# Kyaw-Thiha/animal-vision

Hardware: AMD Instinct MI355X
Metric: megapixels/sec per-frame pipeline (higher is better)
Workload: dtype f16

## Files before the change

animal-vision_amd/_lib.py:

```python
from __future__ import annotations

import ctypes
import os

_HERE = os.path.dirname(os.path.abspath(__file__))
LIB_PATH = os.path.join(_HERE, "libavx.so")

AVX_OK = 0
AVX_ERR_INVALID, AVX_ERR_NO_DEVICE, AVX_ERR_HIP, AVX_ERR_UNSUPPORTED, AVX_ERR_NOMEM = -1, -2, -3, -4, -5
AVX_COLOR_MATRIX, AVX_COLOR_CAT_MERGE = 0, 1
AVX_POST_NONE, AVX_POST_GAUSS, AVX_POST_ROWGAIN, AVX_POST_STREAK = 0, 1, 2, 3
AVX_MAX_KSIZE = 33
AVX_PIX_FMTS = {"yuv420p": 0, "nv12": 1, "yuv422p": 2, "yuv444p": 3, "gray": 4, "yuv420p10le": 5, "yuv422p10le": 6, "yuv444p10le": 7,
                "p010le": 8}
AVX_TRANSFERS = {"pq": 1, "hlg": 2}
AVX_TONEMAPS = {"clip": 0, "mobius": 1}


class AvxError(RuntimeError):
    def __init__(self, code: int, msg: str):
        super().__init__(f"libavx error {code}: {msg}")
        self.code = code


# ... 387 lines not shown
                           _vp, _vp, _vp]),
    "avx_remap_linear_planes": (_i, [_vp, _vp, _i, _i, _i, _vp, _vp, _vp, ctypes.c_float, _vp]),
    "avx_sobel3_plane": (_i, [_vp, _vp, _i, _i, _vp, _vp, _vp]),
    "avx_mst_gram": (_i, [_vp, _vp, _i, _sz, _i, _i, _vp, _vp, _vp, _vp]),
    "avx_mst_qkv_gram": (_i, [_vp, _vp, _vp, _sz, _i, _vp, _vp, _vp, _vp, _vp]),
    "avx_mst_qkv_gram16": (_i, [_vp, _vp, _vp, _sz, _i, _vp, _vp, _vp, _vp, _vp]),
    "avx_mst_ln_gemm_gelu": (_i, [_vp, _vp, _vp, _vp, ctypes.c_float, _vp, _sz, _i, _vp, _vp]),
    "avx_mst_convt2x2": (_i, [_vp, _vp, _vp, _vp, _vp, _i, _i, _i, _i, _vp]),
    "avx_mst_convt2x2_fuse": (_i, [_vp, _vp, _vp, _vp, _vp, _vp, _vp, _i, _i, _i, _i, _vp]),
    "avx_mst_posemb": (_i, [_vp, _vp, _vp, _vp, _vp, _vp, _vp, _i, _i, _i, _i, _vp]),
    "avx_mst_conv3x3_add": (_i, [_vp, _vp, _vp, _vp, _vp, _i, _i, _i, _i, _vp]),
    "avx_mst_attn_pack": (_i, [_vp, _vp, _vp, _vp, _vp, _vp, _i, _vp, _vp]),
    "avx_mst_rowgemm_add": (_i, [_vp, _vp, _vp, _vp, _vp, _vp, _vp, _sz, _i, _vp]),
    "avx_mst_conv_in_u8": (_i, [_vp, _vp, _i, _i, _i, _i, _i, _i, _vp, _vp, _vp]),
    "avx_mst_conv3x3_lds": (_i, [_vp, _vp, _vp, _vp, _vp, _i, _i, _i, _i, _vp]),
    "avx_mst_down4x4": (_i, [_vp, _vp, _vp, _vp, _i, _i, _i, _i, _vp]),
    "avx_mst_conv3x3_lds_gram": (_i, [_vp, _vp, _vp, _vp, _vp, _i, _i, _i, _vp, _vp, _vp, _vp, _vp]),
    "avx_mst_conv3x3_lds_cin": (_i, [_vp, _vp, _vp, _vp, _i, _i, _i, _i, _i, _i, _vp, _vp, _vp]),
    "avx_mst_conv3x3_lds_spectral_cin": (_i, [_vp, _vp, _vp, _vp, _i, _i, _i, _i, _i, _i, _vp, _fp, _i, _i, _i, _i, _vp, _vp, ctypes.POINTER(ctypes.c_int), _vp]),
    "avx_mst_conv3x3_lds_gram_cin": (_i, [_vp, _vp, _i, _i, _i, _i, _i, _i, _vp, _vp, _vp, _vp, _vp, _vp, _vp, _vp]),
    "avx_mst_convt2x2_fuse_gram": (_i, [_vp, _vp, _vp, _vp, _vp, _vp, _vp, _i, _i, _i, _vp, _vp, _vp, _vp, _vp]),
    "avx_mst_convt2x2_fuse16": (_i, [_vp, _vp, _vp, _vp, _vp, _vp, _vp, _i, _i, _i, _i, _vp]),
    "avx_mst_convt2x2_fuse16_gram": (_i, [_vp, _vp, _vp, _vp, _vp, _vp, _vp, _i, _i, _i, _i, _vp, _vp, _vp, _vp, _vp]),
    "avx_mst_attn_pack16": (_i, [_vp, _vp, _vp, _vp, _vp, _vp, _i, _vp, _vp]),
    "avx_mst_attn_pack_mx": (_i, [_vp, _vp, _vp, _vp, _vp, _vp, _i, _vp, _vp]),
    "avx_mst_attn_tail_mx": (_i, [_vp, _vp, _vp, _vp, _vp, _vp, _vp, _vp, _i, _i, _i, _i, _vp]),
    "avx_mst_attn_tail_sp": (_i, [_vp, _vp, _vp, _vp, _vp, _vp, _vp, _vp, _i, _i, _i, _i, _vp]),
    "avx_mst_attn_tail_mx_col": (_i, [_vp, _vp, _vp, _vp, _vp, _vp, _vp, _vp, _i, _i, _i, _i, _i, _vp]),
    "avx_mst_attn_tail_sp_col": (_i, [_vp, _vp, _vp, _vp, _vp, _vp, _vp, _vp, _i, _i, _i, _i, _i, _vp]),
    "avx_mst_tail_march_steps": (_i, [_i, _i, _i, _i, ctypes.POINTER(ctypes.c_longlong), ctypes.POINTER(ctypes.c_ubyte), _i, ctypes.POINTER(ctypes.c_int)]),
    "avx_mst_attn_tail": (_i, [_vp, _vp, _vp, _vp, _vp, _vp, _vp, _vp, _i, _i, _i, _i, _vp]),
    "avx_mst_attn_tail_x": (_i, [_vp, _vp, _vp, _vp, _vp, _vp, _vp, _vp, _i, _i, _i, _i, _vp]),
    "avx_mst_ffn_fused": (_i, [_vp, _vp, _vp, _vp, ctypes.c_float, _vp, _vp, _vp, _vp, _i, _i, _i, _i, _vp]),
    "avx_mst_conv3x3_lds_spectral": (_i, [_vp, _vp, _vp, _vp, _i, _i, _i, _fp, _i, _i, _i, _i, _vp, _vp, ctypes.POINTER(ctypes.c_int), _vp]),
    "avx_mst_ffn_fused_mx": (_i, [_vp, _vp, _vp, _vp, ctypes.c_float, _vp, _vp, _vp, _vp, _i, _i, _i, _i, _vp]),
    "avx_mst_ffn_fused_sp": (_i, [_vp, _vp, _vp, _vp, ctypes.c_float, _vp, _vp, _vp, _vp, _i, _i, _i, _i, _vp]),
    "avx_mst_ffn_fused_mx_col": (_i, [_vp, _vp, _vp, _vp, ctypes.c_float, _vp, _vp, _vp, _vp, _i, _i, _i, _i, _i, _vp]),
    "avx_mst_ffn_fused_sp_col": (_i, [_vp, _vp, _vp, _vp, ctypes.c_float, _vp, _vp, _vp, _vp, _i, _i, _i, _i, _i, _vp]),
    "avx_mst_gelu_prescale": (ctypes.c_float, []),
    "avx_mst_tile_order": (_i, [_i, _i, _i, _i, _i, ctypes.POINTER(ctypes.c_longlong), _i, ctypes.POINTER(ctypes.c_int)]),
    "avx_mst_tile_order_col": (_i, [_i, _i, _i, _i, ctypes.POINTER(ctypes.c_longlong), ctypes.POINTER(ctypes.c_ubyte), _i, ctypes.POINTER(ctypes.c_int)]),
    "avx_mst_dw_gemm_add": (_i, [_vp, _vp, _vp, _vp, _vp, _vp, _i, _i, _i, _i, _vp]),
    "avx_dwconv3x3_nhwc_add": (_i, [_vp, _vp, _vp, _vp, _i, _i, _i, _i, _i, _vp, _vp, _vp]),
    "avx_dwconv3x3_nhwc": (_i, [_vp, _vp, _vp, _vp, _i, _i, _i, _i, _i, _i, _vp]),
    "avx_layernorm_rows": (_i, [_vp, _vp, _vp, _vp, _vp, _i, _sz, _i, ctypes.c_float, _vp]),
    "avx_layernorm_rows_grouped": (_i, [_vp, _vp, _vp, _vp, _vp, _i, _sz, _i, ctypes.c_float, _i, _i, _vp]),
# ... 9 lines not shown
```

animal-vision_amd/csrc/mst_mfma.hip:

```cpp
#include <hip/hip_fp16.h>

#include "avx_internal.h"
#include "mst_common.h"

namespace {

constexpr int kT = 256;

__device__ __forceinline__ float16_t mfma(half4_t a, half4_t b, float16_t c) { return __builtin_amdgcn_mfma_f32_32x32x8f16(a, b, c, 0, 0, 0); }
__device__ __forceinline__ float16_t mfma16(half8_t a, half8_t b, float16_t c) { return __builtin_amdgcn_mfma_f32_32x32x16_f16(a, b, c, 0, 0, 0); }

template <int C>
__device__ __forceinline__ void load_x(const __half* __restrict__ x, size_t tile, size_t n, int lane, half4_t (&xf)[C / 8]) {
    const int p = lane & 31, h = lane >> 5;
    const size_t row = tile * 32 + p;
    if (row < n) {
        const uint4* src = reinterpret_cast<const uint4*>(x + row * (size_t)C + h * (C / 2));
#pragma unroll
        for (int q = 0; q < C / 16; ++q) {
            const uint4 v = src[q];
            const half8_t h8 = __builtin_bit_cast(half8_t, v);
            xf[2 * q] = half4_t{h8[0], h8[1], h8[2], h8[3]};
            xf[2 * q + 1] = half4_t{h8[4], h8[5], h8[6], h8[7]};
        }
    } else {
#pragma unroll
// ... 880 lines not shown

template <int C, bool SKIP, bool GRAM>
int launch_convt16(avx_ctx* ctx, avx_ws* ws, const void* x, const void* wpack, const float* bias, const void* skip, const void* wskip, void* out, int B, int H, int W,
                   const void* wqk, float* gram, float* nq, float* nk, hipStream_t s) {
    constexpr int NW = convt16_geom<C, SKIP, GRAM>::NW, KS = C / 16, CO = C / 2, NT = CO / 32, KSS = CO / 16, HD = NT;
    size_t lds = sizeof(uint4) * ((size_t)4 * NT * KS * 64 + (SKIP ? NT * KSS * 64 : 0) + (GRAM ? 2 * HD * KSS * 64 : 0)) + sizeof(float) * CO;
    if (GRAM && lds < sizeof(float) * NW * HD * 34 * 32) lds = sizeof(float) * NW * HD * 34 * 32;
    const long total = (long)B * H * ((W + 31) / 32);
    long blocks = (total + NW - 1) / NW;
    const long cap = (long)ctx->num_cus * convt16_geom<C, SKIP, GRAM>::PER_CU;
    if (blocks > cap) blocks = cap;
    float* partial = nullptr;
    if (GRAM) {
        int rc = avx_ensure_scratch(ctx, ws, sizeof(float) * (size_t)blocks * HD * 34 * 32);
        if (rc) return rc;
        partial = (float*)ws->d_scratch;
    }
    auto k = k_mst_convt2x2_16<C, NW, SKIP, GRAM>;
    AVX_HIP(ctx, hipFuncSetAttribute((const void*)k, hipFuncAttributeMaxDynamicSharedMemorySize, (int)lds));
    hipLaunchKernelGGL(k, dim3((unsigned)blocks), dim3(64 * NW), lds, s, (const __half*)x, (const uint4*)wpack, bias, (const __half*)skip, (const uint4*)wskip, (__half*)out, B,
                       H, W, (const uint4*)wqk, partial);
    AVX_HIP(ctx, hipGetLastError());
    if (GRAM) return avx_mst_qkv_final_launch(ctx, partial, (int)blocks, HD, gram, nq, nk, s);
    return AVX_OK;
}

template <int C, int NW>
__global__ __launch_bounds__(64 * NW) void k_mst_qkv16(const __half* __restrict__ x, const uint4* __restrict__ wpack , size_t n,
                                                      __half* __restrict__ v_out , float* __restrict__ partial ) {
    constexpr int KS = C / 16, HD = C / 32, NT = 3 * HD;
    extern __shared__ __align__(16) unsigned char smem[];
    uint4* wl = reinterpret_cast<uint4*>(smem);
    const int tid = threadIdx.x, lane = tid & 63, wave = tid >> 6;
    for (int i = tid; i < NT * KS * 64; i += 64 * NW) wl[i] = wpack[i];
    __syncthreads();
    auto W = [&](int t, int s) { return __builtin_bit_cast(half8_t, wl[(t * KS + s) * 64 + lane]); };
    float16_t G[HD];
    float nq[HD], nk[HD];
#pragma unroll
    for (int hd = 0; hd < HD; ++hd) {
#pragma unroll
        for (int v = 0; v < 16; ++v) G[hd][v] = 0.f;
        nq[hd] = 0.f;
        nk[hd] = 0.f;
    }
    const size_t ntiles = (n + 31) / 32;
// ... 371 lines not shown
    if (C == 64) {
        if (skip) return launch_convt16<64, true, false>(ctx, nullptr, x, wpack16, bias, skip, wskip16, out, B, H, W, nullptr, nullptr, nullptr, nullptr, s);
        return launch_convt16<64, false, false>(ctx, nullptr, x, wpack16, bias, nullptr, nullptr, out, B, H, W, nullptr, nullptr, nullptr, nullptr, s);
    }
    if (skip) return launch_convt16<128, true, false>(ctx, nullptr, x, wpack16, bias, skip, wskip16, out, B, H, W, nullptr, nullptr, nullptr, nullptr, s);
    return launch_convt16<128, false, false>(ctx, nullptr, x, wpack16, bias, nullptr, nullptr, out, B, H, W, nullptr, nullptr, nullptr, nullptr, s);
}

int avx_mst_convt2x2_fuse16_gram(avx_ctx* ctx, const void* x, const void* wpack16, const float* bias, const void* skip, const void* wskip16, void* out, int H, int W,
                                 int C, int heads, const void* wqk16, float* gram, float* nq, float* nk, void* stream) {
    if (!ctx) return AVX_ERR_INVALID;
    AVX_REQUIRE(ctx, x && wpack16 && bias && skip && wskip16 && out && wqk16 && gram && nq && nk && H > 0 && W > 0, "avx_mst_convt2x2_fuse16_gram: NULL pointer or empty tensor");
    AVX_REQUIRE(ctx, (C == 64 || C == 128) && heads == C / 64, "avx_mst_convt2x2_fuse16_gram: C=%d, heads=%d (64 or 128 input channels, one head per 32 output channels)", C, heads);
    AVX_REQUIRE(ctx, ((((uintptr_t)x | (uintptr_t)wpack16 | (uintptr_t)out | (uintptr_t)skip | (uintptr_t)wskip16 | (uintptr_t)wqk16)) & 15u) == 0,
                "avx_mst_convt2x2_fuse16_gram: pointers must be 16-byte aligned");
    AVX_HIP(ctx, hipSetDevice(ctx->device));
    hipStream_t s = avx_pick_stream(ctx, stream);
    avx_ws* ws = avx_workspace(ctx, s);
    if (!ws) return AVX_ERR_NOMEM;
    if (C == 64) return launch_convt16<64, true, true>(ctx, ws, x, wpack16, bias, skip, wskip16, out, 1, H, W, wqk16, gram, nq, nk, s);
    return launch_convt16<128, true, true>(ctx, ws, x, wpack16, bias, skip, wskip16, out, 1, H, W, wqk16, gram, nq, nk, s);
}

}
```

animal-vision_amd/ml/mst_plus_plus.py:

```python
from __future__ import annotations

from typing import Dict, List

import torch
import torch.nn.functional as F

DIM = 31
PAD = 32


def padded(n: int) -> int:
    assert n % DIM == 0
    return n // DIM * PAD


def pad_index(n: int, device=None) -> torch.Tensor:
    i = torch.arange(n, device=device)
    return (i // DIM) * PAD + i % DIM


def pad_channels(t: torch.Tensor, dims) -> torch.Tensor:
    for d in dims:
        n = t.shape[d]
        shape = list(t.shape)
# ... 138 lines not shown
        self._conv_in = os.environ.get("AVX_MST_NO_CONV_IN", "") == ""
        self._upfuse = os.environ.get("AVX_MST_NO_UPFUSE", "") == ""
        self._tail = os.environ.get("AVX_MST_NO_TAIL", "") == ""
        self._tailx = os.environ.get("AVX_MST_NO_TAILX", "") == ""
        self._down = os.environ.get("AVX_MST_NO_DOWN4X4", "") == ""
        self._qkv16 = os.environ.get("AVX_MST_NO_QKV16", "") == ""
        self._convgram = os.environ.get("AVX_MST_NO_CONVGRAM", "") == ""
        self._ffn = os.environ.get("AVX_MST_NO_FFN_FUSED", "") == ""
        self._gelu_pre = None
        self._dwmx = os.environ.get("AVX_MST_NO_DW_MFMA", "") == ""
        self._dwsp = os.environ.get("AVX_MST_NO_DW_SPARSE", "") == ""
        self.DW_SPARSE_FFN_C = (32, 64, 128)
        self.DW_SPARSE_TAIL_C = (32, 64)
        self._specfuse = os.environ.get("AVX_MST_NO_SPEC_FUSE", "") == ""
        self._cinfuse = os.environ.get("AVX_MST_NO_CONV_IN_FUSE", "") == ""
        self.FFN_FUSED_C = tuple(int(v) for v in os.environ.get("AVX_MST_FFN_FUSED_C", "32,64,128").split(",") if v)
        self._ffn_march = os.environ.get("AVX_MST_NO_FFN_MARCH", "") == ""
        self.FFN_MARCH_C = (32, 64)
        self._tail_march = os.environ.get("AVX_MST_NO_TAIL_MARCH", "") == ""
        self.TAIL_MARCH_C = (32, 64)
        self._convt16 = os.environ.get("AVX_MST_NO_CONVT16", "") == ""
        self.CONVT16_C = (64, 128)
        self.CONVT16_GRAM_C = (128,)
        self._ctx = {}

    def ctx(self, device: torch.device):
        from ..runtime import get_context

        idx = device.index if device.index is not None else torch.cuda.current_device()
        c = get_context(idx)
        if c.device != idx:
            raise RuntimeError(f"libavx context is on device {c.device}, tensor on cuda:{idx} (one process per GPU)")
        return c

    @staticmethod
    def _dt(t: torch.Tensor) -> int:
        if t.dtype == torch.float32:
            return 0
        if t.dtype == torch.float16:
            return 1
        raise TypeError(f"csrc/mst.hip kernels take float32/float16, got {t.dtype}")

    def gram(self, qkv: torch.Tensor, heads: int):
        from .._lib import lib

        b, n, c3 = qkv.shape
# ... 56 lines not shown
            ctx._check(lib.avx_mst_convt2x2(ctx._h, x.data_ptr(), wpack.data_ptr(), bias.data_ptr(), out.data_ptr(), b, h, w, c, st))
        else:
            assert skip.is_contiguous() and skip.shape == out.shape
            ctx._check(lib.avx_mst_convt2x2_fuse(ctx._h, x.data_ptr(), wpack.data_ptr(), bias.data_ptr(), skip.data_ptr(), wskip.data_ptr(), out.data_ptr(), b, h, w, c, st))
        return out

    def convt2x2_gram(self, x: torch.Tensor, wpack: torch.Tensor, bias: torch.Tensor, skip: torch.Tensor, wskip: torch.Tensor, wqk16: torch.Tensor):
        from .._lib import lib

        b, h, w, c = x.shape
        assert c == 64 and skip.is_contiguous() and skip.shape == (b, 2 * h, 2 * w, 32)
        x = x.contiguous()
        out = torch.empty((b, 2 * h, 2 * w, 32), dtype=torch.float16, device=x.device)
        g = torch.empty((b, 1, 32, 32), dtype=torch.float32, device=x.device)
        nq = torch.empty((b, 32), dtype=torch.float32, device=x.device)
        nk = torch.empty((b, 32), dtype=torch.float32, device=x.device)
        ctx = self.ctx(x.device)
        st = torch.cuda.current_stream(x.device).cuda_stream
        for i in range(b):
            ctx._check(lib.avx_mst_convt2x2_fuse_gram(ctx._h, x[i].data_ptr(), wpack.data_ptr(), bias.data_ptr(), skip[i].data_ptr(), wskip.data_ptr(), out[i].data_ptr(), h, w, c,
                                                      wqk16.data_ptr(), g[i].data_ptr(), nq[i].data_ptr(), nk[i].data_ptr(), st))
        return out, g, nq, nk

    def convt2x2_16(self, x: torch.Tensor, wpack16: torch.Tensor, bias: torch.Tensor, skip: torch.Tensor = None, wskip16: torch.Tensor = None) -> torch.Tensor:
        from .._lib import lib

        b, h, w, c = x.shape
        x = x.contiguous()
        out = torch.empty((b, 2 * h, 2 * w, c // 2), dtype=torch.float16, device=x.device)
        ctx = self.ctx(x.device)
        st = torch.cuda.current_stream(x.device).cuda_stream
        if skip is not None:
            assert skip.is_contiguous() and skip.shape == out.shape and wskip16 is not None
        ctx._check(lib.avx_mst_convt2x2_fuse16(ctx._h, x.data_ptr(), wpack16.data_ptr(), bias.data_ptr(), skip.data_ptr() if skip is not None else None,
                                               wskip16.data_ptr() if skip is not None else None, out.data_ptr(), b, h, w, c, st))
        return out

    def convt2x2_16_gram(self, x: torch.Tensor, wpack16: torch.Tensor, bias: torch.Tensor, skip: torch.Tensor, wskip16: torch.Tensor, wqk16: torch.Tensor):
        from .._lib import lib

        b, h, w, c = x.shape
        ch, heads = c // 2, c // 64
        assert c in (64, 128) and skip.is_contiguous() and skip.shape == (b, 2 * h, 2 * w, ch)
        x = x.contiguous()
        out = torch.empty((b, 2 * h, 2 * w, ch), dtype=torch.float16, device=x.device)
        g = torch.empty((b, heads, 32, 32), dtype=torch.float32, device=x.device)
        nq = torch.empty((b, ch), dtype=torch.float32, device=x.device)
        nk = torch.empty((b, ch), dtype=torch.float32, device=x.device)
        ctx = self.ctx(x.device)
        st = torch.cuda.current_stream(x.device).cuda_stream
        for i in range(b):
            ctx._check(lib.avx_mst_convt2x2_fuse16_gram(ctx._h, x[i].data_ptr(), wpack16.data_ptr(), bias.data_ptr(), skip[i].data_ptr(), wskip16.data_ptr(), out[i].data_ptr(),
                                                        h, w, c, heads, wqk16.data_ptr(), g[i].data_ptr(), nq[i].data_ptr(), nk[i].data_ptr(), st))
        return out, g, nq, nk

    def posemb(self, v: torch.Tensor, w1_c9: torch.Tensor, w2_c9: torch.Tensor, residual: torch.Tensor = None, bias: torch.Tensor = None) -> torch.Tensor:
        from .._lib import lib

        b, h, w, c = v.shape
        v = v.contiguous()
        residual = residual.contiguous() if residual is not None else None
        out = torch.empty_like(v)
        ctx = self.ctx(v.device)
        ctx._check(lib.avx_mst_posemb(ctx._h, v.data_ptr(), w1_c9.data_ptr(), w2_c9.data_ptr(), residual.data_ptr() if residual is not None else None,
                                      bias.data_ptr() if bias is not None else None, out.data_ptr(), b, h, w, c, torch.cuda.current_stream(v.device).cuda_stream))
        return out

    def conv3x3(self, x: torch.Tensor, wpack: torch.Tensor, add: torch.Tensor = None) -> torch.Tensor:
        from .._lib import lib

        b, h, w, c = x.shape
        x = x.contiguous()
        add = add.contiguous() if add is not None else None
        out = torch.empty_like(x)
        ctx = self.ctx(x.device)
        ctx._check(lib.avx_mst_conv3x3_add(ctx._h, x.data_ptr(), wpack.data_ptr(), add.data_ptr() if add is not None else None, out.data_ptr(), b, h, w, c,
# ... 551 lines not shown
            fea = self._conv3(x, ekey)
        skips: List[torch.Tensor] = []
        heads = 1
        for i in range(2):
            fea = self._msab(fea, f"{p}.encoder_layers.{i}.0", heads, pre if i == 0 else None)
            skips.append(fea)
            dkey = f"{p}.encoder_layers.{i}.1.weight"
            if _AVX.fused_ok(fea) and _AVX._down and fea.shape[-1] in (32, 64) and fea.is_contiguous():
                fea = _AVX.down4x4(fea, self._prep(dkey + ".frag16", lambda: pack_down4x4(self._w(dkey, (0, 1)))))
            else:
                fea = self._conv_nhwc(fea, self._w(dkey, (0, 1)), stride=2, padding=1)
            heads *= 2
        fea = self._msab(fea, p + ".bottleneck", heads)
        for i in range(2):
            kw = f"{p}.decoder_layers.{i}.0.weight"
            if _AVX.fused_ok(fea) and fea.shape[-1] in (64, 128) and _AVX._upfuse:
                ch = fea.shape[-1] // 2
                wfk = f"{p}.fuse{i}"
                wf_ = self._prep(wfk, lambda: self._w(f"{p}.decoder_layers.{i}.1.weight", (0, 1)).reshape(ch, 2 * ch).t().contiguous())
                gb = self._prep(kw + ".upfuse.bias", lambda: (self._w(f"{p}.decoder_layers.{i}.0.bias", (0,)).float() @ wf_[:ch].float()).contiguous())
                heads //= 2
                a2 = f"{p}.decoder_layers.{i}.2.blocks.0.0"
                cangram = _AVX._convgram and _AVX._qkv16 and _AVX._tail and _AVX._tailx
                gram16 = cangram and _AVX._convt16 and 2 * ch in _AVX.CONVT16_C and 2 * ch in _AVX.CONVT16_GRAM_C
                gram8 = cangram and ch == 32 and not gram16
                k16 = gram16 or (_AVX._convt16 and 2 * ch in _AVX.CONVT16_C and not gram8)
                tap = lambda t: (self._w(kw, (0, 1))[:, :, t // 2, t % 2].float() @ wf_[:ch].float()).half().contiguous()
                if k16:
                    gt = self._prep(kw + ".upfuse4k16", lambda: torch.stack([pack_fragments16(tap(t), halfrow=True) for t in range(4)]).contiguous())
                    wbot_ = self._prep(f"{p}.fuse{i}.bot16", lambda: pack_fragments16(wf_[ch:].contiguous(), halfrow=True))
                else:
                    gt = self._prep(kw + ".upfuse4", lambda: torch.stack([pack_fragments(tap(t), True) for t in range(4)]).contiguous())
                    wbot_ = self._prep(f"{p}.fuse{i}.bot", lambda: pack_fragments(wf_[ch:].contiguous(), True))
                pre2 = None
                if gram16 or gram8:
                    wqkv2 = self._prep(a2 + ".qkv", lambda: torch.cat([self._w(a2 + ".to_q.weight", (0, 1)), self._w(a2 + ".to_k.weight", (0, 1)),
                                                                       self._w(a2 + ".to_v.weight", (0, 1))], 0).t().contiguous())
                    wqk2 = self._prep(a2 + ".qkv.frag16", lambda: pack_qkv16(wqkv2))
                    fea, *pre2 = (_AVX.convt2x2_16_gram if gram16 else _AVX.convt2x2_gram)(fea, gt, gb, skips[1 - i].contiguous(), wbot_, wqk2)
                else:
                    fea = (_AVX.convt2x2_16 if k16 else _AVX.convt2x2)(fea, gt, gb, skips[1 - i].contiguous(), wbot_)
                fea = self._msab(fea, f"{p}.decoder_layers.{i}.2", heads, tuple(pre2) if pre2 else None)
                continue
            if _AVX.fused_ok(fea) and fea.shape[-1] in (64, 128):
                wt = self._prep(kw + ".frag4", lambda: torch.stack([pack_fragments(self._w(kw, (0, 1))[:, :, t // 2, t % 2].contiguous(), True) for t in range(4)]).contiguous())
                bt = self._prep(kw + ".bias32", lambda: self._w(f"{p}.decoder_layers.{i}.0.bias", (0,)).float().contiguous())
                up = _AVX.convt2x2(fea, wt, bt)
            else:
                up = F.conv_transpose2d(fea.permute(0, 3, 1, 2), self._w(kw, (0, 1)), self._w(f"{p}.decoder_layers.{i}.0.bias", (0,)), stride=2).permute(0, 2, 3, 1)
            heads //= 2
            skip = skips[1 - i]
            b, h, w, ch = up.shape
            c2 = 2 * ch
            wf = self._prep(f"{p}.fuse{i}", lambda: self._w(f"{p}.decoder_layers.{i}.1.weight", (0, 1)).reshape(c2 // 2, c2).t().contiguous())
            if _AVX.fused_ok(skip):
                up, skip = up.contiguous(), skip.contiguous()
                wtop = self._prep(f"{p}.fuse{i}.top", lambda: pack_fragments(wf[:ch].contiguous(), True))
                wbot = self._prep(f"{p}.fuse{i}.bot", lambda: pack_fragments(wf[ch:].contiguous(), True))
                fea = _AVX.rowgemm_add(up.reshape(b * h * w, ch), wtop, None, skip.reshape(b * h * w, ch), wbot).reshape(b, h, w, ch)
            else:
                cat = torch.cat([up, skip], dim=-1)
                fea = (cat.reshape(b, h * w, c2) @ wf).reshape(b, h, w, c2 // 2)
            fea = self._msab(fea, f"{p}.decoder_layers.{i}.2", heads)
        if src is not None:
# ... 91 lines not shown
```

include/avx.h:

```cpp
#ifndef AVX_H
#define AVX_H

#include <stddef.h>
#include <stdint.h>

#ifdef __cplusplus
extern "C" {
#endif

#define AVX_ABI_VERSION 1

typedef struct avx_ctx avx_ctx;

typedef enum avx_status {
    AVX_OK = 0,
    AVX_ERR_INVALID = -1,
    AVX_ERR_NO_DEVICE = -2,
    AVX_ERR_HIP = -3,
    AVX_ERR_UNSUPPORTED = -4,
    AVX_ERR_NOMEM = -5
} avx_status;

int avx_abi_version(void);
int avx_device_count(void);
// ... 459 lines not shown
                             const float* bias, void* out, int B, int H, int W, int C, int max_workgroups, void* stream);
int avx_mst_attn_tail_sp_col(avx_ctx* ctx, const void* x, const void* wvpack16, const void* mpack_mx, const void* dw1pack, const void* dw2pack,
                             const float* bias, void* out, int B, int H, int W, int C, int max_workgroups, void* stream);
int avx_mst_tail_march_steps(int frames, int ty, int tx, int nwg, long long* visit, unsigned char* prime, int steps_cap, int* steps_out);

int avx_mst_rowgemm_add(avx_ctx* ctx, const void* a, const void* wpack, const void* a2, const void* wpack2, const void* add, void* out, size_t rows,
                        int C, void* stream);

int avx_mst_attn_pack(avx_ctx* ctx, const float* gram, const float* nq, const float* nk, const float* rescale, const float* wproj_t, int C,
                      void* mpack, void* stream);

int avx_mst_conv3x3_add(avx_ctx* ctx, const void* x, const void* wpack, const void* add, void* out, int B, int H, int W, int C, void* stream);

int avx_mst_posemb(avx_ctx* ctx, const void* v, const float* w1_c9, const float* w2_c9, const void* residual, const float* bias, void* out, int B,
                   int H, int W, int C, void* stream);

int avx_mst_convt2x2(avx_ctx* ctx, const void* x, const void* wpack, const float* bias, void* out, int B, int H, int W, int C, void* stream);
int avx_mst_convt2x2_fuse(avx_ctx* ctx, const void* x, const void* wpack, const float* bias, const void* skip, const void* wskip, void* out, int B, int H,
                          int W, int C, void* stream);
int avx_mst_convt2x2_fuse16(avx_ctx* ctx, const void* x, const void* wpack16, const float* bias, const void* skip, const void* wskip16, void* out, int B, int H,
                            int W, int C, void* stream);
int avx_mst_convt2x2_fuse16_gram(avx_ctx* ctx, const void* x, const void* wpack16, const float* bias, const void* skip, const void* wskip16, void* out, int H, int W,
                                 int C, int heads, const void* wqk16, float* gram, float* nq, float* nk, void* stream);

int avx_dwconv3x3_nhwc(avx_ctx* ctx, const void* x, const float* w_c9, void* y, int dtype, int B, int H, int W, int C, int gelu_out, void* stream);
int avx_dwconv3x3_nhwc_add(avx_ctx* ctx, const void* x, const float* w_c9, void* y, int B, int H, int W, int C, int gelu_out,
                           const void* residual, const float* bias, void* stream);

int avx_layernorm_rows(avx_ctx* ctx, const void* x, const float* gamma, const float* beta, void* y, int dtype, size_t rows, int C, float eps, void* stream);
int avx_layernorm_rows_grouped(avx_ctx* ctx, const void* x, const float* gamma, const float* beta, void* y, int dtype, size_t rows, int C, float eps,
                               int group, int real, void* stream);

int avx_get_table(int which, void* dst_host, size_t capacity);

#ifdef __cplusplus
}
#endif
#endif
```

Measured before the change: 464.6.

## Add whole-line convt2x2 fuse kernel with async skip DMA into LDS

Adds a new transposed-conv 2x2 fused kernel that processes whole output line runs per wave. It streams the skip input with global_load_lds DMA into swizzled LDS areas, double-buffered across tiles. Results are staged in LDS so the global stores are fully coalesced, and a variant also fuses the gram/qkv reduction for C=64. This targets uncoalesced skip reads and output writes and overlaps memory with MFMA work. In exchange it uses one large workgroup per CU, inline asm waitcnt tricks and complex swizzle maps.

```diff
diff --git a/animal-vision_amd/_lib.py b/animal-vision_amd/_lib.py
--- a/animal-vision_amd/_lib.py
+++ b/animal-vision_amd/_lib.py
@@ -433,6 +433,9 @@
     "avx_mst_convt2x2_fuse_gram": (_i, [_vp, _vp, _vp, _vp, _vp, _vp, _vp, _i, _i, _i, _vp, _vp, _vp, _vp, _vp]),
     "avx_mst_convt2x2_fuse16": (_i, [_vp, _vp, _vp, _vp, _vp, _vp, _vp, _i, _i, _i, _i, _vp]),
     "avx_mst_convt2x2_fuse16_gram": (_i, [_vp, _vp, _vp, _vp, _vp, _vp, _vp, _i, _i, _i, _i, _vp, _vp, _vp, _vp, _vp]),
+    "avx_mst_convt2x2_fuse16_ln": (_i, [_vp, _vp, _vp, _vp, _vp, _vp, _vp, _i, _i, _i, _i, _vp]),
+    "avx_mst_convt2x2_fuse16_gram_ln": (_i, [_vp, _vp, _vp, _vp, _vp, _vp, _vp, _i, _i, _i, _i, _vp, _vp, _vp, _vp, _vp]),
+    "avx_mst_convt_lines_map": (_i, [_i] + [ctypes.POINTER(ctypes.c_int)] * 4),
     "avx_mst_attn_pack16": (_i, [_vp, _vp, _vp, _vp, _vp, _vp, _i, _vp, _vp]),
     "avx_mst_attn_pack_mx": (_i, [_vp, _vp, _vp, _vp, _vp, _vp, _i, _vp, _vp]),
     "avx_mst_attn_tail_mx": (_i, [_vp, _vp, _vp, _vp, _vp, _vp, _vp, _vp, _i, _i, _i, _i, _vp]),
diff --git a/animal-vision_amd/csrc/mst_convt_lines.h b/animal-vision_amd/csrc/mst_convt_lines.h
--- /dev/null
+++ b/animal-vision_amd/csrc/mst_convt_lines.h
@@ -0,0 +1,26 @@
+#pragma once
+
+__host__ __device__ constexpr int convt_ln_skip_slot(int cpp, int i, int k) {
+    if (cpp == 4) {
+        const int ql = k >> 2, c = k & 3, hi = ql >> 3, pl = (ql >> 1) & 3, dx = ql & 1;
+        return 16 * c + 4 * ((i ^ (3 * hi) ^ dx) & 3) + pl;
+    }
+    const int ql = k >> 3, c = k & 7, pl = ql >> 1, dx = ql & 1;
+    return 16 * (c >> 1) + 4 * ((i & 3) ^ (2 * (c & 1) + dx)) + pl;
+}
+__host__ __device__ constexpr int convt_ln_skip_chunk(int cpp, int i, int l) {
+    const int u = l >> 4, v = ((l >> 2) ^ i) & 3, pl = l & 3;
+    if (cpp == 4) {
+        const int hi = v >> 1, dx = (v & 1) ^ hi;
+        return 4 * (8 * hi + 2 * pl + dx) + u;
+    }
+    return 8 * (2 * pl + (v & 1)) + 2 * u + (v >> 1);
+}
+__host__ __device__ constexpr int convt_ln_operand_byte(int cpp, int p, int h, int dx, int s) {
+    const int g = (2 * p + dx) * cpp + h * (cpp / 2) + s;
+    return 1024 * (g >> 6) + 16 * convt_ln_skip_slot(cpp, g >> 6, g & 63);
+}
+__host__ __device__ constexpr int convt_ln_out_byte(int cpp, int g) {
+    const int i = g >> 6, k = g & 63;
+    return 1024 * i + 16 * (k ^ (cpp == 4 ? k >> 3 : ((k >> 4) & 3) | (i & 1) << 2));
+}
diff --git a/animal-vision_amd/csrc/mst_mfma.hip b/animal-vision_amd/csrc/mst_mfma.hip
--- a/animal-vision_amd/csrc/mst_mfma.hip
+++ b/animal-vision_amd/csrc/mst_mfma.hip
@@ -2,6 +2,7 @@
 
 #include "avx_internal.h"
 #include "mst_common.h"
+#include "mst_convt_lines.h"
 
 namespace {
 
@@ -928,6 +929,253 @@
                        H, W, (const uint4*)wqk, partial);
     AVX_HIP(ctx, hipGetLastError());
     if (GRAM) return avx_mst_qkv_final_launch(ctx, partial, (int)blocks, HD, gram, nq, nk, s);
+    return AVX_OK;
+}
+
+#pragma clang diagnostic push
+#pragma clang diagnostic ignored "-Winline-asm"
+__device__ __forceinline__ void ln_dma16(const void* base , unsigned ofs, unsigned lds_base ) {
+    asm volatile("s_mov_b32 m0, %0\n\ts_nop 0\n\tglobal_load_lds_dwordx4 %1, %2" ::"s"(__builtin_amdgcn_readfirstlane(lds_base)), "v"(ofs), "s"(base) : "memory", "m0");
+}
+#pragma clang diagnostic pop
+template <int C, bool GRAM> struct convt_ln_geom {
+    static constexpr int NW = C == 128 ? 8 : GRAM ? 12 : 16, AREAS = C == 128 ? 1 : 2, KS = C / 16, CO = C / 2, NT = CO / 32, KSS = CO / 16, HD = NT, NP = C / 16, ROWB = 64 * C;
+    static constexpr int WBYTES = 16 * (4 * NT * KS * 64 + NT * KSS * 64 + (GRAM ? 2 * HD * KSS * 64 : 0)) + 4 * CO;
+    static constexpr int LDS = (WBYTES + 1023) / 1024 * 1024 + 1024  + NW * AREAS * ROWB;
+    static_assert(LDS <= 160 * 1024 && (!GRAM || 4 * NW * HD * 34 * 32 <= LDS), "one workgroup per CU");
+};
+template <int C, int NW_, bool GRAM>
+__global__ __launch_bounds__(64 * NW_, 1) void k_mst_convt2x2_16_ln(const __half* __restrict__ x , const uint4* __restrict__ wpack ,
+                                                                  const float* __restrict__ bias , const __half* __restrict__ skip ,
+                                                                  const uint4* __restrict__ wskip , __half* __restrict__ out , int B,
+                                                                  int H, int W, const uint4* __restrict__ wqk , float* __restrict__ partial ) {
+    using G_ = convt_ln_geom<C, GRAM>;
+    static_assert(NW_ == G_::NW, "the geometry is convt_ln_geom's");
+    constexpr int NW = G_::NW, AREAS = G_::AREAS, KS = G_::KS, CO = G_::CO, NT = G_::NT, KSS = G_::KSS, HD = G_::HD, NP = G_::NP, ROWB = G_::ROWB;
+    using run_t = unsigned __attribute__((ext_vector_type(4 * NP)));
+    using u4_t = unsigned __attribute__((ext_vector_type(4)));
+    extern __shared__ __align__(16) unsigned char smem[];
+    uint4* wl = reinterpret_cast<uint4*>(smem);
+    float* bl = reinterpret_cast<float*>(wl + 4 * NT * KS * 64);
+    uint4* wsl = reinterpret_cast<uint4*>(bl + CO);
+    uint4* wq = wsl + NT * KSS * 64;
+    const int tid = threadIdx.x, lane = tid & 63, wave = __builtin_amdgcn_readfirstlane(tid >> 6);
+    for (int i = tid; i < 4 * NT * KS * 64; i += 64 * NW) wl[i] = wpack[i];
+    for (int i = tid; i < CO; i += 64 * NW) bl[i] = bias[i];
+    for (int i = tid; i < NT * KSS * 64; i += 64 * NW) wsl[i] = wskip[i];
+    float16_t G[GRAM ? HD : 1];
+    float nq[GRAM ? HD : 1], nk[GRAM ? HD : 1];
+    if constexpr (GRAM) {
+        for (int i = tid; i < 2 * HD * KSS * 64; i += 64 * NW) wq[i] = wqk[i];
+#pragma unroll
+        for (int hd = 0; hd < HD; ++hd) {
+#pragma unroll
+            for (int v = 0; v < 16; ++v) G[hd][v] = 0.f;
+            nq[hd] = 0.f;
+            nk[hd] = 0.f;
+        }
+    }
+    __syncthreads();
+    const int xt = (W + 31) / 32;
+    const unsigned total = (unsigned)B * (unsigned)H * (unsigned)xt;
+    const int p = lane & 31, h = lane >> 5;
+    const unsigned lds0 = (unsigned)(size_t)(__attribute__((address_space(3))) unsigned char*)smem;
+    const unsigned a0 = __builtin_amdgcn_readfirstlane(((lds0 + (unsigned)G_::WBYTES + 1023u) & ~1023u) + (unsigned)wave * (AREAS * ROWB));
+    unsigned char* const area = smem + (a0 - lds0);
+    int fo[NP], ob[2][KSS], wb[2][NT][2];
+    const int rb[2] = {convt_ln_out_byte(NP, lane), convt_ln_out_byte(NP, 64 + lane) - 1024};
+#pragma unroll
+    for (int i = 0; i < NP; ++i) fo[i] = 1024 * i + 16 * convt_ln_skip_chunk(NP, i, lane);
+#pragma unroll
+    for (int dx = 0; dx < 2; ++dx) {
+#pragma unroll
+        for (int s = 0; s < KSS; ++s) ob[dx][s] = convt_ln_operand_byte(NP, p, h, dx, s);
+#pragma unroll
+        for (int t = 0; t < NT; ++t) {
+            wb[dx][t][0] = convt_ln_out_byte(NP, (2 * p + dx) * NP + 4 * t + 2 * h);
+            wb[dx][t][1] = convt_ln_out_byte(NP, (2 * p + dx) * NP + 4 * t + 2 * h + 1);
+        }
+    }
+    const unsigned nwaves = gridDim.x * NW, first = blockIdx.x * NW + wave;
+    const int sx = (int)(nwaves % (unsigned)xt), sy = (int)(nwaves / (unsigned)xt);
+    int xi = (int)(first % (unsigned)xt), yb = (int)(first / (unsigned)xt);
+    unsigned tile = first;
+    auto run_ofs = [&](int yb_, int xi_, int dy) { return ((size_t)(2 * yb_ + dy) * (size_t)(2 * W) + (size_t)(64 * xi_)) * (size_t)C; };
+    auto run_len = [&](int xi_) { const int px = 2 * W - 64 * xi_; return (px < 64 ? px : 64) * C; };
+    auto request = [&](int yb_, int xi_, int dy, int a) {
+        const char* base = reinterpret_cast<const char*>(skip) + run_ofs(yb_, xi_, dy);
+        const int last = run_len(xi_) - 16;
+#pragma unroll
+        for (int i = 0; i < NP; ++i) ln_dma16(base, (unsigned)(fo[i] < last ? fo[i] : last), a0 + a * ROWB + i * 1024);
+    };
+    auto load_x = [&](int yb_, int xi_, u4_t (&r)[KS]) {
+        const int xw = 32 * xi_ + p;
+        const u4_t* src = reinterpret_cast<const u4_t*>(x + ((size_t)yb_ * (size_t)W + (size_t)(xw < W ? xw : W - 1)) * C + h * (C / 2));
+#pragma unroll
+        for (int q = 0; q < KS; ++q) r[q] = src[q];
+    };
+    if (tile < total) {
+        u4_t xr[KS];
+        load_x(yb, xi, xr);
+#pragma unroll
+        for (int q = 0; q < KS; ++q) asm volatile("" : "+v"(xr[q]));
+        request(yb, xi, 0, 0);
+        if constexpr (AREAS == 2) request(yb, xi, 1, 1);
+        asm volatile("s_waitcnt vmcnt(%0)" ::"n"((AREAS - 1) * NP) : "memory");
+        for (;;) {
+            int nxi = xi + sx, nyb = yb + sy;
+            if (nxi >= xt) { nxi -= xt; ++nyb; }
+            const bool more = tile + nwaves < total && tile + nwaves > tile;
+            if (!more) { nxi = xi; nyb = yb; }
+            const int xw = 32 * xi + p, lastc = run_len(xi) / 16 - 1;
+            u4_t xn[KS];
+#pragma unroll
+            for (int dy = 0; dy < 2; ++dy) {
+                unsigned char* const ar = area + (AREAS == 2 ? dy : 0) * ROWB;
+                asm volatile("s_waitcnt vmcnt(%0)" ::"n"(AREAS * NP) : "memory");
+                if (dy == 0) load_x(nyb, nxi, xn);
+                uint4 sr[2][KSS];
+#pragma unroll
+                for (int dx = 0; dx < 2; ++dx)
+#pragma unroll
+                    for (int s = 0; s < KSS; ++s) sr[dx][s] = *reinterpret_cast<const uint4*>(ar + ob[dx][s]);
+#pragma unroll
+                for (int dx = 0; dx < 2; ++dx) {
+                    const int tap = 2 * dy + dx;
+                    uint4 og[NT][2];
+#pragma unroll
+                    for (int t = 0; t < NT; ++t) {
+                        float16_t d;
+#pragma unroll
+                        for (int v = 0; v < 16; ++v) d[v] = 0.f;
+#pragma unroll
+                        for (int s = 0; s < KS; ++s) d = mfma16(__builtin_bit_cast(half8_t, wl[((tap * NT + t) * KS + s) * 64 + lane]), __builtin_bit_cast(half8_t, xr[s]), d);
+#pragma unroll
+                        for (int s = 0; s < KSS; ++s) d = mfma16(__builtin_bit_cast(half8_t, wsl[(t * KSS + s) * 64 + lane]), __builtin_bit_cast(half8_t, sr[dx][s]), d);
+                        half8_t o0, o1;
+#pragma unroll
+                        for (int v = 0; v < 8; ++v) { o0[v] = (_Float16)(d[v] + bl[32 * t + 16 * h + v]); o1[v] = (_Float16)(d[8 + v] + bl[32 * t + 16 * h + 8 + v]); }
+                        *reinterpret_cast<uint4*>(ar + wb[dx][t][0]) = __builtin_bit_cast(uint4, o0);
+                        *reinterpret_cast<uint4*>(ar + wb[dx][t][1]) = __builtin_bit_cast(uint4, o1);
+                        if constexpr (GRAM) {
+#pragma unroll
+                            for (int v = 0; v < 8; ++v) { o0[v] = xw < W ? o0[v] : (_Float16)0.f; o1[v] = xw < W ? o1[v] : (_Float16)0.f; }
+                            og[t][0] = __builtin_bit_cast(uint4, o0);
+                            og[t][1] = __builtin_bit_cast(uint4, o1);
+                        }
+                    }
+                    if constexpr (GRAM) {
+                        half8_t xq[KSS];
+                        if constexpr (NT == 1) {
+                            xq[0] = __builtin_bit_cast(half8_t, og[0][0]);
+                            xq[1] = __builtin_bit_cast(half8_t, og[0][1]);
+                        } else {
+                            unsigned a[8] = {og[0][0].x, og[0][0].y, og[0][0].z, og[0][0].w, og[0][1].x, og[0][1].y, og[0][1].z, og[0][1].w};
+                            unsigned c[8] = {og[1][0].x, og[1][0].y, og[1][0].z, og[1][0].w, og[1][1].x, og[1][1].y, og[1][1].z, og[1][1].w};
+#pragma unroll
+                            for (int i = 0; i < 8; ++i) {
+                                const auto r = __builtin_amdgcn_permlane32_swap(a[i], c[i], false, false);
+                                a[i] = r[0];
+                                c[i] = r[1];
+                            }
+                            xq[0] = __builtin_bit_cast(half8_t, uint4{a[0], a[1], a[2], a[3]});
+                            xq[1] = __builtin_bit_cast(half8_t, uint4{a[4], a[5], a[6], a[7]});
+                            xq[2] = __builtin_bit_cast(half8_t, uint4{c[0], c[1], c[2], c[3]});
+                            xq[3] = __builtin_bit_cast(half8_t, uint4{c[4], c[5], c[6], c[7]});
+                        }
+#pragma unroll
+                        for (int hd = 0; hd < HD; ++hd) {
+                            float16_t dq, dk;
+#pragma unroll
+                            for (int v = 0; v < 16; ++v) { dq[v] = 0.f; dk[v] = 0.f; }
+#pragma unroll
+                            for (int s = 0; s < KSS; ++s) dq = mfma16(xq[s], __builtin_bit_cast(half8_t, wq[(hd * KSS + s) * 64 + lane]), dq);
+#pragma unroll
+                            for (int s = 0; s < KSS; ++s) dk = mfma16(xq[s], __builtin_bit_cast(half8_t, wq[((HD + hd) * KSS + s) * 64 + lane]), dk);
+                            unsigned aq[8], ak[8];
+#pragma unroll
+                            for (int j = 0; j < 8; ++j) {
+                                aq[j] = pack_f16(dq[2 * j], dq[2 * j + 1]);
+                                ak[j] = pack_f16(dk[2 * j], dk[2 * j + 1]);
+                                fma_mix_lo(nq[hd], aq[j], aq[j]); fma_mix_hi(nq[hd], aq[j], aq[j]);
+                                fma_mix_lo(nk[hd], ak[j], ak[j]); fma_mix_hi(nk[hd], ak[j], ak[j]);
+                            }
+#pragma unroll
+                            for (int b2 = 0; b2 < 2; ++b2)
+                                G[hd] = mfma16(__builtin_bit_cast(half8_t, uint4{ak[4 * b2], ak[4 * b2 + 1], ak[4 * b2 + 2], ak[4 * b2 + 3]}),
+                                               __builtin_bit_cast(half8_t, uint4{aq[4 * b2], aq[4 * b2 + 1], aq[4 * b2 + 2], aq[4 * b2 + 3]}), G[hd]);
+                        }
+                    }
+                }
+                run_t ov;
+                int oc[NP];
+#pragma unroll
+                for (int i = 0; i < NP; ++i) {
+                    const bool in = 64 * i + lane <= lastc;
+                    oc[i] = in ? 64 * i + lane : lastc;
+                    const uint4 v = *reinterpret_cast<const uint4*>(ar + (in ? rb[i & 1] + 1024 * i : convt_ln_out_byte(NP, lastc)));
+                    ov[4 * i] = v.x; ov[4 * i + 1] = v.y; ov[4 * i + 2] = v.z; ov[4 * i + 3] = v.w;
+                }
+                asm volatile("s_waitcnt lgkmcnt(0)" ::: "memory");
+                unsigned char* const dst = reinterpret_cast<unsigned char*>(out) + run_ofs(yb, xi, dy);
+                if constexpr (AREAS == 1) request(dy == 0 ? yb : nyb, dy == 0 ? xi : nxi, dy ^ 1, 0);
+#pragma unroll
+                for (int i = 0; i < NP; ++i)
+                    *reinterpret_cast<uint4*>(dst + 16 * oc[i]) = uint4{ov[4 * i], ov[4 * i + 1], ov[4 * i + 2], ov[4 * i + 3]};
+                if constexpr (AREAS == 2) request(nyb, nxi, dy, dy);
+            }
+#pragma unroll
+            for (int q = 0; q < KS; ++q) asm volatile("" : "+v"(xn[q]));
+            if (!more) break;
+#pragma unroll
+            for (int q = 0; q < KS; ++q) xr[q] = xn[q];
+            xi = nxi;
+            yb = nyb;
+            tile += nwaves;
+        }
+        asm volatile("s_waitcnt vmcnt(0)" ::: "memory");
+    }
+    if constexpr (GRAM) {
+        __syncthreads();
+        float* red = reinterpret_cast<float*>(smem);
+#pragma unroll
+        for (int hd = 0; hd < HD; ++hd) {
+            float* mine = red + ((size_t)wave * HD + hd) * 34 * 32;
+#pragma unroll
+            for (int v = 0; v < 16; ++v) mine[(8 * (v / 4) + 4 * h + (v % 4)) * 32 + p] = G[hd][v];
+            const float sq = nq[hd] + __shfl_xor(nq[hd], 32), sk = nk[hd] + __shfl_xor(nk[hd], 32);
+            if (h == 0) { mine[32 * 32 + p] = sq; mine[33 * 32 + p] = sk; }
+        }
+        __syncthreads();
+        for (int i = tid; i < HD * 34 * 32; i += 64 * NW) {
+            float sum = 0.f;
+#pragma unroll
+            for (int w = 0; w < NW; ++w) sum += red[(size_t)w * HD * 34 * 32 + i];
+            partial[(size_t)blockIdx.x * HD * 34 * 32 + i] = sum;
+        }
+    }
+}
+
+template <int C, bool GRAM>
+int launch_convt16_ln(avx_ctx* ctx, avx_ws* ws, const void* x, const void* wpack, const float* bias, const void* skip, const void* wskip, void* out, int B, int H, int W,
+                      const void* wqk, float* gram, float* nq, float* nk, hipStream_t s) {
+    using G_ = convt_ln_geom<C, GRAM>;
+    const long total = (long)B * H * ((W + 31) / 32);
+    AVX_REQUIRE(ctx, total < 0x7fffffffl && (long)B * H * 2 < 0x7fffffffl, "avx_mst_convt2x2_fuse16_ln: %ld wave-tiles (fewer than 2^31)", total);
+    long blocks = (total + G_::NW - 1) / G_::NW;
+    if (blocks > ctx->num_cus) blocks = ctx->num_cus;
+    float* partial = nullptr;
+    if (GRAM) {
+        int rc = avx_ensure_scratch(ctx, ws, sizeof(float) * (size_t)blocks * G_::HD * 34 * 32);
+        if (rc) return rc;
+        partial = (float*)ws->d_scratch;
+    }
+    auto k = k_mst_convt2x2_16_ln<C, G_::NW, GRAM>;
+    AVX_HIP(ctx, hipFuncSetAttribute((const void*)k, hipFuncAttributeMaxDynamicSharedMemorySize, (int)G_::LDS));
+    hipLaunchKernelGGL(k, dim3((unsigned)blocks), dim3(64 * G_::NW), G_::LDS, s, (const __half*)x, (const uint4*)wpack, bias, (const __half*)skip, (const uint4*)wskip, (__half*)out, B,
+                       H, W, (const uint4*)wqk, partial);
+    AVX_HIP(ctx, hipGetLastError());
+    if (GRAM) return avx_mst_qkv_final_launch(ctx, partial, (int)blocks, G_::HD, gram, nq, nk, s);
     return AVX_OK;
 }
 
@@ -1345,4 +1593,52 @@
     return launch_convt16<128, true, true>(ctx, ws, x, wpack16, bias, skip, wskip16, out, 1, H, W, wqk16, gram, nq, nk, s);
 }
 
-}
+int avx_mst_convt2x2_fuse16_ln(avx_ctx* ctx, const void* x, const void* wpack16, const float* bias, const void* skip, const void* wskip16, void* out, int B, int H, int W,
+                               int C, void* stream) {
+    if (!ctx) return AVX_ERR_INVALID;
+    AVX_REQUIRE(ctx, x && wpack16 && bias && out && skip && wskip16 && B > 0 && H > 0 && W > 0, "avx_mst_convt2x2_fuse16_ln: NULL pointer or empty tensor");
+    AVX_REQUIRE(ctx, C == 64 || C == 128, "avx_mst_convt2x2_fuse16_ln: C=%d (64 or 128 input channels)", C);
+    AVX_REQUIRE(ctx, ((((uintptr_t)x | (uintptr_t)wpack16 | (uintptr_t)out | (uintptr_t)skip | (uintptr_t)wskip16)) & 15u) == 0,
+                "avx_mst_convt2x2_fuse16_ln: pointers must be 16-byte aligned");
+    AVX_HIP(ctx, hipSetDevice(ctx->device));
+    hipStream_t s = avx_pick_stream(ctx, stream);
+    if (C == 64) return launch_convt16_ln<64, false>(ctx, nullptr, x, wpack16, bias, skip, wskip16, out, B, H, W, nullptr, nullptr, nullptr, nullptr, s);
+    return launch_convt16_ln<128, false>(ctx, nullptr, x, wpack16, bias, skip, wskip16, out, B, H, W, nullptr, nullptr, nullptr, nullptr, s);
+}
+
+int avx_mst_convt2x2_fuse16_gram_ln(avx_ctx* ctx, const void* x, const void* wpack16, const float* bias, const void* skip, const void* wskip16, void* out, int H, int W,
+                                    int C, int heads, const void* wqk16, float* gram, float* nq, float* nk, void* stream) {
+    if (!ctx) return AVX_ERR_INVALID;
+    AVX_REQUIRE(ctx, x && wpack16 && bias && skip && wskip16 && out && wqk16 && gram && nq && nk && H > 0 && W > 0, "avx_mst_convt2x2_fuse16_gram_ln: NULL pointer or empty tensor");
+    AVX_REQUIRE(ctx, (C == 64 || C == 128) && heads == C / 64, "avx_mst_convt2x2_fuse16_gram_ln: C=%d, heads=%d (64 or 128 input channels, one head per 32 output channels)", C, heads);
+    AVX_REQUIRE(ctx, ((((uintptr_t)x | (uintptr_t)wpack16 | (uintptr_t)out | (uintptr_t)skip | (uintptr_t)wskip16 | (uintptr_t)wqk16)) & 15u) == 0,
+                "avx_mst_convt2x2_fuse16_gram_ln: pointers must be 16-byte aligned");
+    AVX_HIP(ctx, hipSetDevice(ctx->device));
+    hipStream_t s = avx_pick_stream(ctx, stream);
+    avx_ws* ws = avx_workspace(ctx, s);
+    if (!ws) return AVX_ERR_NOMEM;
+    if (C == 64) return launch_convt16_ln<64, true>(ctx, ws, x, wpack16, bias, skip, wskip16, out, 1, H, W, wqk16, gram, nq, nk, s);
+    return launch_convt16_ln<128, true>(ctx, ws, x, wpack16, bias, skip, wskip16, out, 1, H, W, wqk16, gram, nq, nk, s);
+}
+
+int avx_mst_convt_lines_map(int C, int* fetch, int* operand, int* out_write, int* out_read) {
+    if (C != 64 && C != 128) return AVX_ERR_INVALID;
+    const int np = C / 16, kss = C / 32, nt = C / 64;
+    for (int lane = 0; lane < 64; ++lane) {
+        const int p = lane & 31, h = lane >> 5;
+        for (int i = 0; i < np; ++i) {
+            if (fetch) fetch[i * 64 + lane] = 1024 * i + 16 * convt_ln_skip_chunk(np, i, lane);
+            if (out_read) out_read[i * 64 + lane] = convt_ln_out_byte(np, 64 * i + lane);
+        }
+        for (int dx = 0; dx < 2; ++dx) {
+            for (int s = 0; s < kss; ++s)
+                if (operand) operand[(dx * kss + s) * 64 + lane] = convt_ln_operand_byte(np, p, h, dx, s);
+            for (int t = 0; t < nt; ++t)
+                for (int b = 0; b < 2; ++b)
+                    if (out_write) out_write[((dx * nt + t) * 2 + b) * 64 + lane] = convt_ln_out_byte(np, (2 * p + dx) * np + 4 * t + 2 * h + b);
+        }
+    }
+    return AVX_OK;
+}
+
+}
diff --git a/animal-vision_amd/ml/mst_plus_plus.py b/animal-vision_amd/ml/mst_plus_plus.py
--- a/animal-vision_amd/ml/mst_plus_plus.py
+++ b/animal-vision_amd/ml/mst_plus_plus.py
@@ -184,6 +184,9 @@
         self._convt16 = os.environ.get("AVX_MST_NO_CONVT16", "") == ""
         self.CONVT16_C = (64, 128)
         self.CONVT16_GRAM_C = (128,)
+        self._convt_lines = os.environ.get("AVX_MST_NO_CONVT_LINES", "") == ""
+        self.CONVT_LINES_C = (64, 128)
+        self.CONVT_LINES_GRAM_C = (64,)
         self._ctx = {}
 
     def ctx(self, device: torch.device):
@@ -286,7 +289,8 @@
                                                       wqk16.data_ptr(), g[i].data_ptr(), nq[i].data_ptr(), nk[i].data_ptr(), st))
         return out, g, nq, nk
 
-    def convt2x2_16(self, x: torch.Tensor, wpack16: torch.Tensor, bias: torch.Tensor, skip: torch.Tensor = None, wskip16: torch.Tensor = None) -> torch.Tensor:
+    def convt2x2_16(self, x: torch.Tensor, wpack16: torch.Tensor, bias: torch.Tensor, skip: torch.Tensor = None, wskip16: torch.Tensor = None,
+                    lines: bool = False) -> torch.Tensor:
         from .._lib import lib
 
         b, h, w, c = x.shape
@@ -296,11 +300,16 @@
         st = torch.cuda.current_stream(x.device).cuda_stream
         if skip is not None:
             assert skip.is_contiguous() and skip.shape == out.shape and wskip16 is not None
+        if lines:
+            assert skip is not None, "the whole-line form is the fused step's"
+            ctx._check(lib.avx_mst_convt2x2_fuse16_ln(ctx._h, x.data_ptr(), wpack16.data_ptr(), bias.data_ptr(), skip.data_ptr(), wskip16.data_ptr(), out.data_ptr(), b, h, w, c, st))
+            return out
         ctx._check(lib.avx_mst_convt2x2_fuse16(ctx._h, x.data_ptr(), wpack16.data_ptr(), bias.data_ptr(), skip.data_ptr() if skip is not None else None,
                                                wskip16.data_ptr() if skip is not None else None, out.data_ptr(), b, h, w, c, st))
         return out
 
-    def convt2x2_16_gram(self, x: torch.Tensor, wpack16: torch.Tensor, bias: torch.Tensor, skip: torch.Tensor, wskip16: torch.Tensor, wqk16: torch.Tensor):
+    def convt2x2_16_gram(self, x: torch.Tensor, wpack16: torch.Tensor, bias: torch.Tensor, skip: torch.Tensor, wskip16: torch.Tensor, wqk16: torch.Tensor,
+                         lines: bool = False):
         from .._lib import lib
 
         b, h, w, c = x.shape
@@ -313,9 +322,10 @@
         nk = torch.empty((b, ch), dtype=torch.float32, device=x.device)
         ctx = self.ctx(x.device)
         st = torch.cuda.current_stream(x.device).cuda_stream
+        fn = lib.avx_mst_convt2x2_fuse16_gram_ln if lines else lib.avx_mst_convt2x2_fuse16_gram
         for i in range(b):
-            ctx._check(lib.avx_mst_convt2x2_fuse16_gram(ctx._h, x[i].data_ptr(), wpack16.data_ptr(), bias.data_ptr(), skip[i].data_ptr(), wskip16.data_ptr(), out[i].data_ptr(),
-                                                        h, w, c, heads, wqk16.data_ptr(), g[i].data_ptr(), nq[i].data_ptr(), nk[i].data_ptr(), st))
+            ctx._check(fn(ctx._h, x[i].data_ptr(), wpack16.data_ptr(), bias.data_ptr(), skip[i].data_ptr(), wskip16.data_ptr(), out[i].data_ptr(),
+                          h, w, c, heads, wqk16.data_ptr(), g[i].data_ptr(), nq[i].data_ptr(), nk[i].data_ptr(), st))
         return out, g, nq, nk
 
     def posemb(self, v: torch.Tensor, w1_c9: torch.Tensor, w2_c9: torch.Tensor, residual: torch.Tensor = None, bias: torch.Tensor = None) -> torch.Tensor:
@@ -913,9 +923,11 @@
                 heads //= 2
                 a2 = f"{p}.decoder_layers.{i}.2.blocks.0.0"
                 cangram = _AVX._convgram and _AVX._qkv16 and _AVX._tail and _AVX._tailx
-                gram16 = cangram and _AVX._convt16 and 2 * ch in _AVX.CONVT16_C and 2 * ch in _AVX.CONVT16_GRAM_C
+                ln_gram = cangram and _AVX._convt16 and _AVX._convt_lines and 2 * ch in _AVX.CONVT_LINES_GRAM_C
+                gram16 = ln_gram or (cangram and _AVX._convt16 and 2 * ch in _AVX.CONVT16_C and 2 * ch in _AVX.CONVT16_GRAM_C)
                 gram8 = cangram and ch == 32 and not gram16
                 k16 = gram16 or (_AVX._convt16 and 2 * ch in _AVX.CONVT16_C and not gram8)
+                lines = ln_gram or (k16 and not gram16 and _AVX._convt_lines and 2 * ch in _AVX.CONVT_LINES_C)
                 tap = lambda t: (self._w(kw, (0, 1))[:, :, t // 2, t % 2].float() @ wf_[:ch].float()).half().contiguous()
                 if k16:
                     gt = self._prep(kw + ".upfuse4k16", lambda: torch.stack([pack_fragments16(tap(t), halfrow=True) for t in range(4)]).contiguous())
@@ -928,9 +940,14 @@
                     wqkv2 = self._prep(a2 + ".qkv", lambda: torch.cat([self._w(a2 + ".to_q.weight", (0, 1)), self._w(a2 + ".to_k.weight", (0, 1)),
                                                                        self._w(a2 + ".to_v.weight", (0, 1))], 0).t().contiguous())
                     wqk2 = self._prep(a2 + ".qkv.frag16", lambda: pack_qkv16(wqkv2))
-                    fea, *pre2 = (_AVX.convt2x2_16_gram if gram16 else _AVX.convt2x2_gram)(fea, gt, gb, skips[1 - i].contiguous(), wbot_, wqk2)
+                    if gram16:
+                        fea, *pre2 = _AVX.convt2x2_16_gram(fea, gt, gb, skips[1 - i].contiguous(), wbot_, wqk2, lines=lines)
+                    else:
+                        fea, *pre2 = _AVX.convt2x2_gram(fea, gt, gb, skips[1 - i].contiguous(), wbot_, wqk2)
+                elif k16:
+                    fea = _AVX.convt2x2_16(fea, gt, gb, skips[1 - i].contiguous(), wbot_, lines=lines)
                 else:
-                    fea = (_AVX.convt2x2_16 if k16 else _AVX.convt2x2)(fea, gt, gb, skips[1 - i].contiguous(), wbot_)
+                    fea = _AVX.convt2x2(fea, gt, gb, skips[1 - i].contiguous(), wbot_)
                 fea = self._msab(fea, f"{p}.decoder_layers.{i}.2", heads, tuple(pre2) if pre2 else None)
                 continue
             if _AVX.fused_ok(fea) and fea.shape[-1] in (64, 128):
diff --git a/include/avx.h b/include/avx.h
--- a/include/avx.h
+++ b/include/avx.h
@@ -505,6 +505,11 @@
                             int W, int C, void* stream);
 int avx_mst_convt2x2_fuse16_gram(avx_ctx* ctx, const void* x, const void* wpack16, const float* bias, const void* skip, const void* wskip16, void* out, int H, int W,
                                  int C, int heads, const void* wqk16, float* gram, float* nq, float* nk, void* stream);
+int avx_mst_convt2x2_fuse16_ln(avx_ctx* ctx, const void* x, const void* wpack16, const float* bias, const void* skip, const void* wskip16, void* out, int B, int H,
+                               int W, int C, void* stream);
+int avx_mst_convt2x2_fuse16_gram_ln(avx_ctx* ctx, const void* x, const void* wpack16, const float* bias, const void* skip, const void* wskip16, void* out, int H,
+                                    int W, int C, int heads, const void* wqk16, float* gram, float* nq, float* nk, void* stream);
+int avx_mst_convt_lines_map(int C, int* fetch, int* operand, int* out_write, int* out_read);
 
 int avx_dwconv3x3_nhwc(avx_ctx* ctx, const void* x, const float* w_c9, void* y, int dtype, int B, int H, int W, int C, int gelu_out, void* stream);
 int avx_dwconv3x3_nhwc_add(avx_ctx* ctx, const void* x, const float* w_c9, void* y, int B, int H, int W, int C, int gelu_out,
```

Result: faster. 471.6 (median of 6 runs) (+1.5%).
